# erick093/MPI_Pytorch

Hardware: AMD Instinct MI355X
Metric: images/sec (whole node) ResNet-18 224x224 training at 1/2/4/8 MI355X (higher is better)
Workload: dtype bf16; 1 GPU; model=resnet18, global_batch=2048, per_gpu_batch=2048, image_size=224, num_classes=64500, optimizer=adam, parallelism=dp1, device=cuda, backend=none, hip_graph=False, deterministic=True

## Files before the change

csrc/bindings.cpp:

```cpp
#include <torch/extension.h>
#include <c10/hip/HIPStream.h>
#include <c10/core/DeviceGuard.h>

#include <vector>

#include "kernels/api.h"
#include "runtime/runtime.h"

using torch::Tensor;

namespace {

inline hipStream_t cur_stream() { return c10::hip::getCurrentHIPStream().stream(); }

#define CHECK_CUDA(x) TORCH_CHECK((x).is_cuda(), #x " must be a GPU tensor")
#define CHECK_CONTIG(x) TORCH_CHECK((x).is_contiguous(), #x " must be contiguous")
#define CHECK_BF16(x) \
  TORCH_CHECK((x).scalar_type() == torch::kBFloat16, #x " must be bfloat16, got ", (x).scalar_type())
#define CHECK_F32(x) \
  TORCH_CHECK((x).scalar_type() == torch::kFloat32, #x " must be float32, got ", (x).scalar_type())
#define CHECK_ACT(x) \
  CHECK_CUDA(x);     \
  CHECK_CONTIG(x);   \
  CHECK_BF16(x)
// ... 198 lines not shown
      if (Hp <= 0 || Wp <= 0) continue;
      const int t0 = T;
      for (int r = 0; r < R; ++r) {
        if (((a_ + ph - r) % sh) != 0) continue;
        for (int s = 0; s < S; ++s) {
          if (((b_ + pw - s) % sw) != 0) continue;
          a.taps.dh[T] = (a_ + ph - r) / sh;
          a.taps.dw[T] = (b_ + pw - s) / sw;
          a.taps.bt[T] = r * S + s;
          ++T;
        }
      }
      if (src2) {
        const int R2 = src2->w2.size(1), S2 = src2->w2.size(2);
        for (int r = 0; r < R2; ++r) {
          if (((a_ + src2->ph2 - r) % sh) != 0) continue;
          for (int s = 0; s < S2; ++s) {
            if (((b_ + src2->pw2 - s) % sw) != 0) continue;
            TORCH_CHECK(T < mpa::MAXT, "conv_dgrad: too many taps");
            a.taps.dh[T] = (a_ + src2->ph2 - r) / sh;
            a.taps.dw[T] = (b_ + src2->pw2 - s) / sw;
            a.taps.bt[T] = (short)((r * S2 + s) | mpa::TAP_SRC2);
            ++T;
          }
        }
      }
      TORCH_CHECK(nph < mpa::MAXPH, "conv_dgrad: too many stride phases");
      a.ph[nph++] = mpa::PhaseDesc{N * Hp * Wp, Hp, Wp, (T - t0) * K, t0, T - t0, a_, b_, 0};
    }
  if (bnred) {
    a.ep_z = bp(bnred->z);
    a.ep_y = bopt(bnred->y);
    a.ep_mean = fopt(bnred->mean);
    a.ep_rstd = fopt(bnred->rstd);
    a.ep_gamma = fopt(bnred->gamma);
    a.ep_beta = fopt(bnred->beta);
    TORCH_CHECK(a.ep_y || (a.ep_gamma && a.ep_beta),
                "conv_dgrad_bnred: needs y or gamma / beta for the ReLU mask");
    TORCH_CHECK(!a.ep_gamma == !a.ep_beta, "conv_dgrad_bnred: gamma and beta go together");
    for (const Tensor* t : {&bnred->mean, &bnred->rstd, &bnred->gamma, &bnred->beta})
      TORCH_CHECK(!has(*t) || t->numel() == C, "conv_dgrad_bnred: per-channel vector size");
    bnred->sums = torch::empty({2 * C}, dy.options().dtype(torch::kFloat32));
    int k = 0;
    bool empty = false;
    for (int i = 0; i < nph; ++i) {
      empty |= a.ph[i].T == 0;
      if (a.ph[i].T > 0) a.ph[k++] = a.ph[i];
    }
    if (empty) dx.zero_();
    if (sh == 1 && sw == 1) {
      const mpa::PhaseDesc& d = a.ph[0];
      a.M = d.M; a.oH = d.oH; a.oW = d.oW; a.T = d.T; a.Ktot = d.Ktot; a.Poh = 0; a.Pow = 0;
      a.nphase = 0;
    } else {
      a.nphase = k;
    }
    TORCH_CHECK(!empty, "conv_dgrad_bnred: stride-phase without taps");
    Tensor slab = torch::empty({mpa::igemm_bnred_slab_floats(N * H * W, C, std::max(a.nphase, 1))},
                               dy.options().dtype(torch::kFloat32));
    mpa::igemm_rows_dgrad_bnred(a, vw, bkc, slab.data_ptr<float>(),
                                bnred->sums.data_ptr<float>(), cur_stream());
    return dx;
  }
  if (sh == 1 && sw == 1) {
    const mpa::PhaseDesc& d = a.ph[0];
    a.M = d.M; a.oH = d.oH; a.oW = d.oW; a.T = d.T; a.Ktot = d.Ktot; a.Poh = 0; a.Pow = 0;
    Tensor ws;
    float* wsp = alloc_ws(ws, dy, mpa::igemm_ws_floats(a.M, a.N, a.Ktot));
    mpa::igemm_rows_dgrad(a, vw, wsp, cur_stream(), bkc);
  } else {
    bool empty = false;
    for (int i = 0; i < nph; ++i) empty |= a.ph[i].T == 0;
    int k = 0;
    for (int i = 0; i < nph; ++i)
      if (a.ph[i].T > 0) a.ph[k++] = a.ph[i];
    a.nphase = k;
    if (src2) {
      a.A2 = bp(src2->dy2);
      a.B2 = bp(src2->wt2);
      a.ldb2 = src2->w2.size(1) * src2->w2.size(2) * K;
      if (!mpa::igemm_dgrad_src2_ok(a, vw, bkc)) return Tensor();
    }
    if (empty && !acc) dx.zero_();
    mpa::igemm_rows_dgrad_phases(a, vw, cur_stream(), bkc);
  }
  return dx;
}

Tensor conv_dgrad(Tensor dy, Tensor w, int64_t H, int64_t W, int64_t sh, int64_t sw, int64_t ph,
                  int64_t pw, c10::optional<Tensor> wt_opt, c10::optional<Tensor> accum) {
  return conv_dgrad_impl(dy, w, H, W, sh, sw, ph, pw, wt_opt, nullptr, accum);
}

c10::optional<Tensor> conv_dgrad_res(Tensor dy, Tensor w, Tensor wt, int64_t H, int64_t W,
                                     int64_t ph, int64_t pw, Tensor res, Tensor rmask) {
  CHECK_ACT(dy);
  CHECK_ACT(w);
  CHECK_ACT(res);
  const int N = dy.size(0), P = dy.size(1), Q = dy.size(2), K = dy.size(3);
  const int R = w.size(1), S = w.size(2), C = w.size(3);
  TORCH_CHECK(w.size(0) == K, "conv_dgrad_res: channel mismatch");
  TORCH_CHECK(res.dim() == 4 && res.size(0) == N && res.size(1) == H && res.size(2) == W &&
                  res.size(3) == C,
              "conv_dgrad_res: the residual gradient must have dx's shape");
  TORCH_CHECK(rmask.scalar_type() == torch::kUInt8 && rmask.is_contiguous() &&
                  rmask.numel() == res.numel() / 8 && rmask.device() == res.device(),
              "conv_dgrad_res: ReLU mask must be contiguous uint8 [numel / 8]");
  if (!(wt.defined() && wt.numel() == w.numel()) || vec_width(K) != 8 || vec_width(C) != 8 ||
      mpa::igemm_engine() < 1)
    return c10::nullopt;
  if (P != H + 2 * ph - R + 1 || Q != W + 2 * pw - S + 1) return c10::nullopt;
  if (C % 64 != 0) return c10::nullopt;
  const c10::OptionalDeviceGuard g(device_of(dy));
  Tensor dx = empty_like_shape(dy, {N, H, W, C}, torch::kBFloat16);
  mpa::IGemmArgs a{};
  a.A = bp(dy); a.aH = P; a.aW = Q; a.aC = K;
  a.Uh = 1; a.Uw = 1; a.Oh = 0; a.Ow = 0;
  a.B = bp(wt); a.N = C; a.RS = R * S; a.ldb = R * S * K; a.b_tapmap = 1;
  a.C = dx.data_ptr(); a.ldc = C;
  a.dH = H; a.dW = W; a.Uoh = 1; a.Uow = 1;
  a.beta = 1;
  a.ep_res = bp(res);
  a.ep_rmask = rmask.data_ptr<uint8_t>();
  int T = 0;
  for (int r = 0; r < R; ++r)
    for (int s = 0; s < S; ++s) {
      a.taps.dh[T] = ph - r;
      a.taps.dw[T] = pw - s;
      a.taps.bt[T] = r * S + s;
      ++T;
    }
  a.T = T;
  a.M = N * H * W; a.oH = H; a.oW = W; a.Ktot = T * K; a.Poh = 0; a.Pow = 0;
  if (!mpa::conv3_halo_ok(a)) return c10::nullopt;
  mpa::igemm_rows_dgrad(a, 8, nullptr, cur_stream(), true);
  return dx;
}

c10::optional<Tensor> conv_dgrad_pair(Tensor dy, Tensor w, Tensor wt, int64_t H, int64_t W,
                                      int64_t sh, int64_t sw, int64_t ph, int64_t pw,
                                      Tensor dy2, Tensor w2, Tensor wt2, int64_t ph2,
                                      int64_t pw2, c10::optional<Tensor> accum) {
  CHECK_ACT(dy2);
  CHECK_ACT(w2);
  CHECK_ACT(wt2);
  TORCH_CHECK(dy2.sizes() == dy.sizes(), "conv_dgrad_pair: dy2 must have dy's shape");
  TORCH_CHECK(w2.dim() == 4 && w2.size(0) == w.size(0) && w2.size(3) == w.size(3) &&
                  wt2.numel() == w2.numel(),
              "conv_dgrad_pair: w2 [K][R2][S2][C] with w's K and C, and its transpose");
  if (sh == 1 && sw == 1) return c10::nullopt;
  if (!(wt.defined() && wt.numel() == w.numel())) return c10::nullopt;
  const int P2 = (H + 2 * ph2 - w2.size(1)) / sh + 1, Q2 = (W + 2 * pw2 - w2.size(2)) / sw + 1;
  if (P2 != dy.size(1) || Q2 != dy.size(2)) return c10::nullopt;
  DgradSrc2 s2{dy2, w2, wt2, (int)ph2, (int)pw2};
  Tensor dx = conv_dgrad_impl(dy, w, H, W, sh, sw, ph, pw, wt, nullptr, accum, &s2);
  if (!dx.defined()) return c10::nullopt;
  return dx;
}

bool conv_bnred_ok(int64_t K, int64_t C) {
  return mpa::igemm_engine() >= 1 && vec_width(K) == 8 && vec_width(C) == 8 && C % 8 == 0;
}

std::vector<Tensor> conv_dgrad_bnred(Tensor dy, Tensor w, int64_t H, int64_t W, int64_t sh,
                                     int64_t sw, int64_t ph, int64_t pw, Tensor wt, Tensor z,
                                     Tensor y, Tensor mean, Tensor rstd,
                                     c10::optional<Tensor> gamma, c10::optional<Tensor> beta) {
// ... 1413 lines not shown
  const int64_t ld = src.size(-1);
  TORCH_CHECK(off >= 0 && cs > 0 && off + cs <= ld && (ld * u) % 8 == 0 && (cs * u) % 8 == 0 &&
                  (off * u) % 8 == 0, "chan_slice: 16-byte aligned channel runs required");
  const int64_t rows = src.numel() / ld;
  TORCH_CHECK(rows * (cs * u / 8) < (int64_t(1) << 31), "chan_slice: too large");
  const c10::OptionalDeviceGuard gd(device_of(src));
  std::vector<int64_t> shape(src.sizes().begin(), src.sizes().end());
  shape.back() = cs;
  Tensor out = torch::empty(shape, src.options());
  if (rows > 0)
    mpa::chan_slice((const mpa::bf16_raw*)src.data_ptr(), (int)(ld * u), (int)(off * u),
                    (mpa::bf16_raw*)out.data_ptr(), (int)(cs * u), (int)rows, cur_stream());
  return out;
}

Tensor chan_extract(Tensor g, int64_t off, int64_t cs) {
  CHECK_CUDA(g);
  CHECK_CONTIG(g);
  CHECK_F32(g);
  const int64_t ctot = g.size(-1);
  TORCH_CHECK(ctot % 8 == 0 && cs % 8 == 0 && off % 8 == 0 && off >= 0 && off + cs <= ctot && cs > 0,
              "chan_extract: channel range outside G (multiples of 8 required)");
  const int64_t pixels = g.numel() / ctot;
  TORCH_CHECK(pixels * (cs / 8) < (int64_t(1) << 31), "chan_extract: too large");
  const c10::OptionalDeviceGuard gd(device_of(g));
  std::vector<int64_t> shape(g.sizes().begin(), g.sizes().end());
  shape.back() = cs;
  Tensor out = torch::empty(shape, g.options().dtype(torch::kBFloat16));
  if (pixels > 0)
    mpa::chan_extract(g.data_ptr<float>(), (int)ctot, (int)off, bpm(out), (int)cs, (int)pixels,
                      cur_stream());
  return out;
}

std::vector<Tensor> split_channels(Tensor dy, std::vector<int64_t> sizes) {
  CHECK_ACT(dy);
  TORCH_CHECK(dy.dim() >= 2 && !sizes.empty(), "split_channels: dy must be [..., C]");
  int64_t ctot = 0;
  for (int64_t c : sizes) {
    TORCH_CHECK(c > 0 && c % 8 == 0, "split_channels: channels must be a multiple of 8");
    ctot += c;
  }
  TORCH_CHECK(ctot == dy.size(-1), "split_channels: sizes do not sum to C");
  const int64_t pixels = dy.numel() / ctot;
  TORCH_CHECK(pixels * (ctot / 8) < (int64_t(1) << 31), "split_channels: too large");
  const c10::OptionalDeviceGuard g(device_of(dy));
  std::vector<Tensor> out;
  std::vector<mpa::bf16_raw*> ptrs;
  std::vector<int> chans;
  std::vector<int64_t> shape(dy.sizes().begin(), dy.sizes().end());
  for (int64_t c : sizes) {
    shape.back() = c;
    out.push_back(torch::empty(shape, dy.options()));
    ptrs.push_back(bpm(out.back()));
    chans.push_back((int)c);
  }
  if (pixels > 0)
    mpa::split_channels(bp(dy), chans.data(), (int)sizes.size(), (int)pixels, (int)ctot,
                        ptrs.data(), cur_stream());
  return out;
}

}

extern "C" const char* mpa_src_hash();

PYBIND11_MODULE(TORCH_EXTENSION_NAME, m) {
  m.doc() = "mpi_pytorch_amd native gfx950 kernels + runtime";
  m.def("src_hash", [] { return std::string(mpa_src_hash()); },
        "hash of the csrc/ sources this binary was built from (setup.py source_hash)");
  m.def("igemm_engine", &mpa::igemm_engine, "GEMM staging engine: 1 LDS-DMA, 0 register");
  m.def("igemm_set_engine", &mpa::igemm_set_engine);
  m.def("igemm_force_tile", &mpa::igemm_force_tile, "override GEMM tile (BM, BN, splits); 0 = auto");
  m.def("igemm_set_tune", &mpa::igemm_set_tune, "tile autotuner on/off (MPA_TUNE)");
  m.def("igemm_set_tune_drain", &mpa::igemm_set_tune_drain,
        "tuner candidates: drain the whole device (1, single GPU) or only their stream (0)");
  m.def("set_deterministic", &mpa::set_deterministic,
        "fixed-order reductions + no timing-based autotuning (MPA_DETERMINISTIC)");
  m.def("deterministic", &mpa::deterministic);
  m.def("igemm_tuned_table", &mpa::igemm_tuned_table, "autotuned GEMM tiles so far");
  m.def("igemm_tuned_load", &mpa::igemm_tuned_load, py::arg("table"), py::arg("replace") = true,
        "adopt an igemm_tuned_table() dump (data-parallel ranks take rank 0's)");
  m.def("igemm_set_dma_uni", &mpa::igemm_set_dma_uni, "LDS-DMA uniform-tap fast path on/off");
  m.def("igemm_set_halo", &mpa::igemm_set_halo, "halo-staged direct 3x3/s1 conv on/off");
  m.def("igemm_set_halo_mi7", &mpa::igemm_set_halo_mi7, "448-pixel halo tiles on/off");
  m.def("igemm_set_halo_strip", &mpa::igemm_set_halo_strip,
        "strip-tiled halo conv: 0 off, 1 images too wide for linear tiles, 2 also layer1");
  m.def("igemm_halo_enabled", &mpa::igemm_halo_enabled);
  m.def("igemm_set_stem", &mpa::igemm_set_stem, "direct row-staged 7x7 pixel-pair stem on/off");
  m.def("preprocess_set_copy", &mpa::preprocess_set_copy,
        "identity-size preprocess fast path on/off (MPA_PRE_COPY)");
  m.def("set_comm_reserve", &mpa::set_comm_reserve,
        "CUs held by an overlapping collective (persistent conv grids use the rest)");
  m.def("comm_reserve", &mpa::comm_reserve, "current collective CU reservation");
  m.def("active_cus", &mpa::active_cus, "CUs the persistent conv grids size for");
  m.def("igemm_set_halo_wprod", &mpa::igemm_set_halo_wprod,
        "halo weight gradients on producer-wave blocks on/off (MPA_HALO_WPROD)");
  m.def("igemm_set_halo_wxmap", &mpa::igemm_set_halo_wxmap,
        "XCD-grouped halo weight-gradient block order on/off (MPA_HALO_WXMAP)");
  m.def("igemm_set_halo_trim", &mpa::igemm_set_halo_trim,
        "geometry-sized halo fetch of the linear-tile 3x3 kernels on/off (A/B, tests)");
  m.def("conv3_halo_dma_count", &mpa::conv3_halo_dma_count, py::arg("H"), py::arg("W"),
        "planned halo DMAs per producer wave and item, 256-pixel forward / dgrad tiles");
  m.def("conv3_halo_wgrad_dma_count", &mpa::conv3_halo_wgrad_dma_count, py::arg("H"),
        py::arg("W"), "planned halo DMAs per wave and chunk, 4-wave weight-gradient tiles");
  m.def("affine_act", &affine_act, "relu?(x * aff[0] + aff[1]) per channel (aff [2, C])");
  m.def("conv_fwd", &conv_fwd, py::arg("x"), py::arg("w"), py::arg("bias"), py::arg("sh"),
        py::arg("sw"), py::arg("ph"), py::arg("pw"), py::arg("relu"), py::arg("stats"),
        py::arg("shift"), "conv forward (+ BN statistics of its output)");
  m.def("conv_dgrad", &conv_dgrad, py::arg("dy"), py::arg("w"), py::arg("H"), py::arg("W"),
        py::arg("sh"), py::arg("sw"), py::arg("ph"), py::arg("pw"), py::arg("wt") = py::none(),
        py::arg("accum") = py::none());
  m.def("conv_wgrad", &conv_wgrad, py::arg("dy"), py::arg("x"), py::arg("dw"), py::arg("sh"),
        py::arg("sw"), py::arg("ph"), py::arg("pw"), py::arg("overwrite") = false,
        "weight gradient into dw (+=; overwrite: dw = ..., the first gradient since zero)");
  m.def("conv_bnred_ok", &conv_bnred_ok);
  m.def("conv_dgrad_bnred_gacc", &conv_dgrad_bnred_gacc);
  m.def("conv_dgrad_res", &conv_dgrad_res);
  m.def("conv_dgrad_pair", &conv_dgrad_pair, py::arg("dy"), py::arg("w"), py::arg("wt"),
        py::arg("H"), py::arg("W"), py::arg("sh"), py::arg("sw"), py::arg("ph"), py::arg("pw"),
        py::arg("dy2"), py::arg("w2"), py::arg("wt2"), py::arg("ph2"), py::arg("pw2"),
        py::arg("accum") = py::none());
  m.def("bn_defer_step", &bn_defer_step, py::arg("sums"), py::arg("gamma"), py::arg("mean"),
        py::arg("rstd"), py::arg("s0"), py::arg("k12"), py::arg("dgamma"), py::arg("dbeta"),
        py::arg("G"), py::arg("x"), py::arg("out") = py::none());
  m.def("conv_fwd_into", &conv_fwd_into);
  m.def("conv_dgrad_bnred", &conv_dgrad_bnred, py::arg("dy"), py::arg("w"), py::arg("H"),
        py::arg("W"), py::arg("sh"), py::arg("sw"), py::arg("ph"), py::arg("pw"), py::arg("wt"),
        py::arg("z"), py::arg("y"), py::arg("mean"), py::arg("rstd"),
        py::arg("gamma") = py::none(), py::arg("beta") = py::none());
  m.def("bn_bwd_apply", &bn_bwd_apply);
  m.def("act_bwd", &act_bwd);
  m.def("bn_fwd_train", &bn_fwd_train, py::arg("x"), py::arg("stats"), py::arg("gamma"),
        py::arg("beta"), py::arg("rmean"), py::arg("rvar"), py::arg("momentum"), py::arg("eps"),
        py::arg("res"), py::arg("relu"), py::arg("counter") = py::none(),
        py::arg("mask") = py::none(), py::arg("channels") = 0,
        py::arg("res_affine") = py::none(), py::arg("out") = py::none());
  m.def("bn_stats_affine", &bn_stats_affine, py::arg("x"), py::arg("stats"), py::arg("gamma"),
        py::arg("beta"), py::arg("rmean"), py::arg("rvar"), py::arg("momentum"),
        py::arg("eps"), py::arg("counter") = py::none());
  m.def("bn_stats", &bn_stats, "[mean | biased var] of x [..., C]");
  m.def("bn_relu_avgpool2_fwd", &bn_relu_avgpool2_fwd);
  m.def("bn_fwd_eval", &bn_fwd_eval, py::arg("x"), py::arg("gamma"), py::arg("beta"),
        py::arg("rmean"), py::arg("rvar"), py::arg("eps"), py::arg("res"), py::arg("relu"),
        py::arg("channels") = 0);
  m.def("bn_bwd_pair", &bn_bwd_pair);
  m.def("maxpool_bwd_relu", &maxpool_bwd_relu);
  m.def("bn_bwd", &bn_bwd, py::arg("dy"), py::arg("x"), py::arg("y"), py::arg("mean"),
        py::arg("rstd"), py::arg("gamma"), py::arg("dgamma"), py::arg("dbeta"),
        py::arg("want_dx"), py::arg("want_g"), py::arg("zmask_beta") = py::none(),
        py::arg("ymask") = py::none(), py::arg("gacc") = py::none(),
        py::arg("dx_out") = py::none());
  m.def("relu_fwd", &relu_fwd);
  m.def("comm_emulator", &comm_emulator, "diagnostics: occupy CUs like a concurrent collective");
  m.def("atomic_latency", &atomic_latency, "diagnostics: dependent atomic round trips");
  m.def("maxpool_fwd", &maxpool_fwd);
  m.def("maxpool_bwd", &maxpool_bwd);
  m.def("bn_relu_maxpool_fwd", &bn_relu_maxpool_fwd, py::arg("z"), py::arg("stats"),
        py::arg("gamma"), py::arg("beta"), py::arg("rmean"), py::arg("rvar"), py::arg("momentum"),
        py::arg("eps"), py::arg("kh"), py::arg("kw"), py::arg("sh"), py::arg("sw"), py::arg("ph"),
        py::arg("pw"), py::arg("ceil"), py::arg("counter") = py::none(),
        py::arg("zsel_out") = py::none());
  m.def("maxpool_bn_bwd_sums", &maxpool_bn_bwd_sums);
  m.def("stem_pool_wgrad_ok", &stem_pool_wgrad_ok);
  m.def("stem_pool_wgrad", &stem_pool_wgrad);
  m.def("maxpool_bn_bwd", &maxpool_bn_bwd, py::arg("dp"), py::arg("idx"), py::arg("z"),
// ... 68 lines not shown
```

csrc/kernels/api.h:

```cpp
#pragma once
#include <algorithm>
#include <string>
#include <hip/hip_runtime.h>
#include <stdint.h>

namespace mpa {

typedef uint16_t bf16_raw;
constexpr int MAXT = 128;

struct Taps {
  short dh[MAXT];
  short dw[MAXT];
  short bt[MAXT];
};

struct FastDiv {
  uint32_t m, s;
};
inline FastDiv make_fastdiv(uint32_t d) {
  if (d <= 1) return FastDiv{0u, 0u};
  const uint32_t l = 32u - (uint32_t)__builtin_clz(d - 1u);
  return FastDiv{(uint32_t)(((1ull << (31 + l)) + d - 1) / d), l - 1u};
}

constexpr int MAXPH = 16;
struct PhaseDesc {
  int M, oH, oW, Ktot, tap0, T, Poh, Pow, tiles;
  FastDiv fd_hw, fd_ow;
};

struct IGemmArgs {
  const bf16_raw* A;
  int aH, aW, aC;
  int oH, oW;
  int M;
  int Uh, Uw, Oh, Ow;
  int T;
  int Ktot;
  const bf16_raw* B;
  int N;
  int RS;
  int ldb;
  void* C;
  int ldc;
  int dH, dW, Uoh, Uow, Poh, Pow;
  const float* bias;
  float* stats;
  const float* stats_shift;
  float* stats_sums;
  int stats_ld;
  int relu;
  int ktiles_per_split;
  int tiles_n;
  int tiles_total;
  Taps taps;
  int nphase;
  PhaseDesc ph[MAXPH];
  int b_tapmap;
  int ep_bnred;
  const bf16_raw* ep_z;
  const bf16_raw* ep_y;
  const float* ep_mean;
  const float* ep_rstd;
  const float* ep_gamma;
  const float* ep_beta;
  void* ep_gacc;
  int ep_gacc_f32;
  int stap;
  int beta;
  FastDiv fd_hw, fd_ow;
  const bf16_raw* A2;
  const bf16_raw* B2;
  int ldb2;
  int kpad;
  const bf16_raw* ep_res;
  const uint8_t* ep_rmask;
};
constexpr short TAP_SRC2 = 0x2000;

inline void igemm_set_fastdiv(IGemmArgs& a) {
  a.fd_hw = make_fastdiv((uint32_t)std::max(1, a.oH * a.oW));
  a.fd_ow = make_fastdiv((uint32_t)std::max(1, a.oW));
  for (int i = 0; i < a.nphase && i < MAXPH; ++i) {
    a.ph[i].fd_hw = make_fastdiv((uint32_t)std::max(1, a.ph[i].oH * a.ph[i].oW));
    a.ph[i].fd_ow = make_fastdiv((uint32_t)std::max(1, a.ph[i].oW));
  }
}

struct WGradArgs {
  const bf16_raw* dy;
  const bf16_raw* x;
  float* dw;
  float* slab;
  int Kout, C, H, W, P, Q, R, S, sh, sw, ph, pw;
  int Mpix;
  int Ncols;
  int ktiles_per_split;
  int tiles_n, tiles_total;
  int overwrite;
};

int64_t igemm_slab_floats(int M, int N);
void igemm_rows(IGemmArgs a, int vw, float* ws, float* slab, hipStream_t s);
void igemm_rows_dgrad(IGemmArgs a, int vw, float* ws, hipStream_t s, bool bkc = false);
void igemm_rows_dgrad_phases(IGemmArgs a, int vw, hipStream_t s, bool bkc = false);
bool igemm_dgrad_src2_ok(const IGemmArgs& a, int vw, bool bkc);
int64_t igemm_bnred_slab_floats(int M, int N, int nphase);
void igemm_rows_dgrad_bnred(IGemmArgs a, int vw, bool bkc, float* slab, float* sums,
                            hipStream_t s);
void igemm_wgrad(WGradArgs a, int vwa, int vwb, hipStream_t s);
int64_t igemm_ws_floats(int M, int N, int Ktot);
int64_t igemm_wgrad_ws_floats(int Kout, int Ncols, int Mpix);
int igemm_engine();
void igemm_set_engine(int engine);
void igemm_force_tile(int bm, int bn, int splits);
void igemm_set_tune(int on);
void igemm_set_tune_drain(int on);
std::string igemm_tuned_table();
int igemm_tuned_load(const std::string& table, bool replace);
void igemm_set_dma_uni(int on);
bool igemm_stap_ok();
bool conv3_halo_ok(const IGemmArgs& a);
int conv3_halo(IGemmArgs a, hipStream_t s);
constexpr int HALO_MAX_ROWS = 256;
void igemm_set_halo(int on);
void igemm_set_halo_mi7(int on);
void igemm_set_halo_strip(int mode);
bool stem_wgrad_ok(const WGradArgs& a);
int stem_wgrad(WGradArgs a, hipStream_t s);
int64_t stem_wgrad_ws_floats();
struct StemPoolArgs {
  const bf16_raw* dp;
  const uint8_t* idx;
  const float *mean, *rstd, *gamma, *beta;
  const float* sums;
  int PP, PQ;
  float invM;
};
bool stem_pool_wgrad_ok(const WGradArgs& a, const StemPoolArgs& q);
int stem_pool_wgrad(WGradArgs a, StemPoolArgs q, hipStream_t s);
void igemm_stem_pool_wgrad(WGradArgs a, StemPoolArgs q, hipStream_t s);
bool conv3_halo_wgrad_ok(const WGradArgs& a);
void igemm_set_halo_wxmap(int on);
void igemm_set_halo_wprod(int on);
void igemm_set_halo_trim(int on);
int conv3_halo_dma_count(int H, int W);
int conv3_halo_wgrad_dma_count(int H, int W);
int conv3_halo_wgrad(WGradArgs a, hipStream_t s);
int64_t conv3_halo_wgrad_ws_floats(int Kout, int Ncols);
bool igemm_halo_enabled();
void set_comm_reserve(int cus);
int comm_reserve();
int active_cus();
bool conv_stem_ok(const IGemmArgs& a);
int conv_stem(IGemmArgs a, hipStream_t s);
void igemm_set_stem(int on);

int64_t bn_ws_floats(int M, int C);
void slab_reduce(const float* slab, int S, int W, float* out, bool zero_out, hipStream_t s);
bool dense_gacc_ok(const IGemmArgs& a);
void dense_gacc(IGemmArgs a, float* slab, float* sums, hipStream_t s);
void bn_defer_step(const float* sums, const float* gamma, const float* mean, const float* rstd,
                   int Ci, int s0, int M, float* k12, int ldk, float* dgamma, float* dbeta,
                   void* G, bool g_f32, int ldg, const bf16_raw* x, int ldx, bf16_raw* out,
                   hipStream_t s);
void set_deterministic(int on);
bool deterministic();
void slab_stats(float* slab, int S, int C, const float* shift, int M, float* sums, float* out,
                hipStream_t s, int out_ld = 0);
void stats_finalize(const float* sums, const float* shift, int M, int C, float* out,
                    hipStream_t s);
void bn_stats(const bf16_raw* x, int M, int C, const float* shift, float* stats, float* ws,
              hipStream_t s);
void bn_fwd_train(const bf16_raw* x, const float* stats, const float* gamma, const float* beta,
                  float* rmean, float* rvar, float momentum, float eps, const bf16_raw* res,
                  int relu, int M, int C, bf16_raw* y, float* mean, float* rstd,
                  int64_t* counter, hipStream_t s,
                  uint8_t* ymask = nullptr,
                  int ldx = 0,
                  int lds = 0,
                  const float* res_aff = nullptr,
                  int ldy = 0);
void bn_stats_affine(const float* stats, const float* gamma, const float* beta, float* rmean,
                     float* rvar, float momentum, float eps, int M, int C, float* mean,
                     float* rstd, float* aff, int64_t* counter, hipStream_t s);
void bn_relu_avgpool2_fwd(const bf16_raw* z, const float* aff, int N, int H, int W, int C,
                          bf16_raw* y, hipStream_t s);
void affine_act(const bf16_raw* x, const float* aff, int relu, int M, int C, bf16_raw* y,
                hipStream_t s);
// ... 188 lines not shown
```

csrc/kernels/igemm.hip:

```cpp
#include <algorithm>
#include <cstdio>
#include <cstdlib>
#include <map>
#include <mutex>
#include <string>
#include "igemm_common.h"

namespace mpa {

template <int BM, int BN, int WM, int WN, int VW, bool BKC, bool SPLIT, int OCC>
__global__ __launch_bounds__(256, OCC) void igemm_rows_kernel(IGemmArgs p) {
  constexpr int NA = BM / 64;
  constexpr int A_BYTES = BM * 64;
  constexpr int B_BYTES = BN * 64;
  constexpr int STAGE = A_BYTES + B_BYTES;
  constexpr int TM = BM / WM / 16;
  constexpr int TN = BN / WN / 16;
  constexpr int NB_KC = (BN * 4 + 255) / 256;
  constexpr int CPR = BN / 8;
  constexpr int NB_MN = (BK * CPR + 255) / 256;
  constexpr int NB = BKC ? NB_KC : NB_MN;
  __shared__ __attribute__((aligned(16))) char smem[2 * STAGE];

  const int tid = threadIdx.x;
// ... 855 lines not shown
  a.ep_bnred = 1;
  a.stats = slab;
  a.stats_sums = sums;
  int BM, BN, rows;
  if (a.nphase == 0 && bkc) {
    IGemmArgs t = a;
    if (t.ep_gamma && t.ep_beta) t.ep_y = nullptr;
    if (conv3_halo_ok(t)) {
      rows = conv3_halo(t, s);
      slab_reduce(slab, rows, 2 * a.N, sums, false, s);
      return;
    }
  }
  if (a.nphase > 0) {
    rows = plan_phases(a, BM, BN);
  } else {
    int splits;
    rows_plan(a, BM, BN, splits, false, true);
    rows = (a.M + BM - 1) / BM;
  }
  igemm_rows_dma(a, BM, BN, bkc, 1, s);
  slab_reduce(slab, rows, 2 * a.N, sums, false, s);
}

bool igemm_dgrad_src2_ok(const IGemmArgs& a, int vw, bool bkc) {
  return use_dma(vw) && a.nphase > 0 && a.nphase <= MAXPH && igemm_rows_uni_src2_ok(a, bkc);
}

void igemm_rows_dgrad_phases(IGemmArgs a, int vw, hipStream_t s, bool bkc) {
  a.stats = nullptr;
  a.bias = nullptr;
  if (a.nphase <= 0) return;
  if (a.A2 && !igemm_dgrad_src2_ok(a, vw, bkc)) {
    fprintf(stderr, "igemm_rows_dgrad_phases: second source on an ineligible launch\n");
    abort();
  }
  if (use_dma(vw) && a.nphase <= MAXPH) {
    int tbm = 0, tbn = 0;
    if (g_tune && !deterministic() && !(g_force_bm && g_force_bn) && !stream_capturing(s)) {
      const std::string key = rows_key(a, bkc, false);
      std::unique_lock<std::mutex> pass(g_tune_pass_mu, std::defer_lock);
      if (!tuned_lookup(key, tbm, tbn) && (pass.lock(), !tuned_lookup(key, tbm, tbn))) {
        const int64_t hw0 = std::max(1, a.ph[0].oH * a.ph[0].oW);
        const int64_t rows = (a.ph[0].M + hw0 - 1) / hw0 * a.dH * a.dW;
        const int64_t cbytes = rows * std::max(a.ldc, a.N) * 2;
        char* scr = tune_scratch(cbytes + 256);
        float best = 1e30f;
        for (const auto& c : kRowsCands) {
          if (!scr || !rows_cand_ok(c[0], c[1], a.N)) continue;
          IGemmArgs b = a;
          int BM, BN;
          plan_phases(b, BM, BN, c[0], c[1]);
          if (BM != c[0] || BN != c[1] || b.tiles_total <= 0) continue;
          b.C = scr;
          const float t = time_launches([&] { igemm_rows_dma(b, BM, BN, bkc, 1, s); }, s);
          if (t < best) { best = t; tbm = c[0]; tbn = c[1]; }
        }
        if (tbm) tuned_store(key, tbm, tbn);
      }
    }
    int BM, BN;
    plan_phases(a, BM, BN, tbm, tbn);
    if (a.tiles_total > 0 && igemm_rows_dma(a, BM, BN, bkc, 1, s)) return;
  }
  if (a.A2) {
    fprintf(stderr, "igemm_rows_dgrad_phases: no merged launch for a second source\n");
    abort();
  }
  for (int i = 0; i < a.nphase; ++i) {
    const PhaseDesc& d = a.ph[i];
    IGemmArgs b = a;
    b.nphase = 0;
    b.M = d.M; b.oH = d.oH; b.oW = d.oW; b.Ktot = d.Ktot; b.T = d.T;
    b.Poh = d.Poh; b.Pow = d.Pow;
    for (int t = 0; t < d.T; ++t) {
      b.taps.dh[t] = a.taps.dh[d.tap0 + t];
      b.taps.dw[t] = a.taps.dw[d.tap0 + t];
      b.taps.bt[t] = a.taps.bt[d.tap0 + t];
    }
    run_rows(b, bkc, vw, nullptr, nullptr, s);
  }
}

template <int BM, int BN, int WM, int WN, int VWA, int VWB>
static void launch_wgrad(const WGradArgs& a, int splits, hipStream_t s) {
  dim3 grid(a.tiles_total, 1, splits);
  const int o = occ_target();
  if (o == 4)
    hipLaunchKernelGGL((igemm_wgrad_kernel<BM, BN, WM, WN, VWA, VWB, 4>), grid, dim3(256), 0, s, a);
  else if (o == 2)
    hipLaunchKernelGGL((igemm_wgrad_kernel<BM, BN, WM, WN, VWA, VWB, 2>), grid, dim3(256), 0, s, a);
  else
    hipLaunchKernelGGL((igemm_wgrad_kernel<BM, BN, WM, WN, VWA, VWB, 3>), grid, dim3(256), 0, s, a);
}

template <int BM, int BN>
static void wgrad_vw(const WGradArgs& a, int vwa, int vwb, int splits, hipStream_t s) {
  if (vwb == 1) {
    if (vwa == 8) launch_wgrad<BM, BN, 2, 2, 8, 1>(a, splits, s);
    else if (vwa == 4) launch_wgrad<BM, BN, 2, 2, 4, 1>(a, splits, s);
    else launch_wgrad<BM, BN, 2, 2, 1, 1>(a, splits, s);
  } else {
    if (vwa == 8) launch_wgrad<BM, BN, 2, 2, 8, 8>(a, splits, s);
    else if (vwa == 4) launch_wgrad<BM, BN, 2, 2, 4, 8>(a, splits, s);
    else launch_wgrad<BM, BN, 2, 2, 1, 8>(a, splits, s);
  }
}

static bool wgrad_big(const WGradArgs& a, bool dma_ok) {
  return dma_ok && (a.Kout >= 256 || ((int64_t)a.Kout * a.Ncols <= 32768 && a.Mpix >= (1 << 20)));
}

static bool wgrad_tile_ok(int bm, int bn, bool dma) {
  const bool ok_reg = (bm == 64 || bm == 128) && bn == 128;
  const bool ok_dma = ok_reg || (bn == 256 && (bm == 64 || bm == 128 || bm == 256));
  return dma ? ok_dma : ok_reg;
}

static void wgrad_plan(WGradArgs& a, int& BM, int& BN, int& splits, bool dma, bool big,
                       int tbm = 0, int tbn = 0) {
  BM = (a.Kout <= 64) ? 64 : 128;
  BN = 128;
  if (dma && BM == 128 && ((a.Kout + 127) / 128) * ((a.Ncols + 127) / 128) < 4) BM = 64;
  if (big) BN = 256, BM = (a.Kout <= 64) ? 64 : 128;
  const bool tuned = tbm && tbn && wgrad_tile_ok(tbm, tbn, dma);
  if (tuned) { BM = tbm; BN = tbn; }
  if (g_force_bm && g_force_bn && wgrad_tile_ok(g_force_bm, g_force_bn, dma)) {
    BM = g_force_bm;
    BN = g_force_bn;
  }
  a.tiles_n = (a.Ncols + BN - 1) / BN;
  const int tiles_m = (a.Kout + BM - 1) / BM;
  a.tiles_total = tiles_m * a.tiles_n;
  const int ktiles = (a.Mpix + BK - 1) / BK;
  const bool stem2 = big && BM == 64 && BN == 256 && !(g_force_bm && g_force_bn) && !tuned &&
                     a.Ncols > 128 && a.Ncols <= 256;
  if (stem2) {
    BN = 128;
    a.tiles_n = (a.Ncols + BN - 1) / BN;
    a.tiles_total = tiles_m * a.tiles_n;
  }
  splits = std::max(1, ((stem2 ? 1024 : 512) + a.tiles_total - 1) / a.tiles_total);
  splits = std::min(splits, std::max(1, ktiles / 16));
  if (g_force_splits > 0) splits = std::min(g_force_splits, std::max(ktiles, 1));
  const int64_t out = (int64_t)a.Kout * a.Ncols;
  splits = (int)std::min<int64_t>(splits, std::max<int64_t>(1, (16ll << 20) / out));
  finish_split_plan(ktiles, splits, a.ktiles_per_split);
}

int64_t igemm_wgrad_ws_floats(int Kout, int Ncols, int Mpix) {
  int64_t best = conv3_halo_wgrad_ws_floats(Kout, Ncols);
  if (Kout == 64 && Ncols == 224) best = std::max(best, stem_wgrad_ws_floats());
  for (int dma = 0; dma < 3; ++dma) {
    WGradArgs a{};
    a.Kout = Kout; a.Ncols = Ncols; a.Mpix = Mpix;
    int BM, BN, splits;
    wgrad_plan(a, BM, BN, splits, dma >= 1, dma == 2);
    if (splits > 1) best = std::max(best, (int64_t)splits * Kout * Ncols);
  }
  return best;
}

static void wgrad_run_plan(WGradArgs a, int vwa, int vwb, hipStream_t s, int tbm, int tbn);

void igemm_stem_pool_wgrad(WGradArgs a, StemPoolArgs q, hipStream_t s) {
  const int z = stem_pool_wgrad(a, q, s);
// ... 94 lines not shown
```

csrc/kernels/igemm_common.h:

```cpp
#pragma once
#include "common.h"
#include "api.h"

namespace mpa {

__device__ __forceinline__ u32x4 u32x4_make(uint32_t a, uint32_t b, uint32_t c, uint32_t d) {
  return u32x4{a, b, c, d};
}

constexpr int BK = 32;

__device__ __forceinline__ int kc_off(int row, int chunk) {
  return row * 64 + ((chunk ^ ((4 - ((row >> 2) & 3)) & 3)) << 4);
}

template <int COLS>
__device__ __forceinline__ int mn_swz(int k) {
  if constexpr (COLS >= 128) return 2 * ((k & 3) | (((k >> 3) & 1) << 2));
  else if constexpr (COLS == 64) return 2 * (((k >> 1) & 1) | (((k >> 3) & 1) << 1));
  else return 2 * ((k >> 3) & 1);
}
template <int COLS>
__device__ __forceinline__ int mn_off(int k, int col) {
  const int chunk = col >> 3;
// ... 289 lines not shown
      }
    }
    if (p.stats) {
#pragma unroll
      for (int j = 0; j < TN; ++j)
#pragma unroll
        for (int r = 0; r < 4; ++r) {
          float a = s[j][r], b = q[j][r];
#pragma unroll
          for (int o = 1; o < 16; o <<= 1) {
            a += __shfl_xor(a, o, 64);
            b += __shfl_xor(b, o, 64);
          }
          s[j][r] = a;
          q[j][r] = b;
        }
      float* red = (float*)smem;
      if ((lane & 15) == 0) {
#pragma unroll
        for (int j = 0; j < TN; ++j) {
          const int col = wcol0 + j * 16 + nl;
#pragma unroll
          for (int r = 0; r < 4; ++r) {
            red[(wm * BN + col + r) * 2] = s[j][r];
            red[(wm * BN + col + r) * 2 + 1] = q[j][r];
          }
        }
      }
      __syncthreads();
      if (stat_row == 0 && block_split() == 0 && tid < BN && n0 + tid < p.N) {
        p.stats_sums[n0 + tid] = 0.f;
        p.stats_sums[p.N + n0 + tid] = 0.f;
      }
      if (tid < BN && n0 + tid < p.N) {
        float a = 0.f, b = 0.f;
#pragma unroll
        for (int w = 0; w < WM; ++w) {
          a += red[(w * BN + tid) * 2];
          b += red[(w * BN + tid) * 2 + 1];
        }
        p.stats[(size_t)stat_row * 2 * p.N + n0 + tid] = a;
        p.stats[(size_t)stat_row * 2 * p.N + p.N + n0 + tid] = b;
      }
    }
  }
}

template <int BM, int BN, int WM, int WN>
__device__ __forceinline__ void wgrad_epilogue(const WGradArgs& p,
                                               f32x4 (&acc)[BM / WM / 16][BN / WN / 16],
                                               int m0, int n0, int wrow0, int wcol0,
                                               int lane) {
  constexpr int TM = BM / WM / 16;
  constexpr int TN = BN / WN / 16;
  const int nl = (lane >> 4) * 4;
  const bool direct = gridDim.z == 1;
  const bool vec = (p.Ncols & 3) == 0;
  float* dst = direct ? p.dw : p.slab + (size_t)blockIdx.z * p.Kout * p.Ncols;
#pragma unroll
  for (int i = 0; i < TM; ++i) {
    const int m = m0 + wrow0 + i * 16 + (lane & 15);
    if (m >= p.Kout) continue;
#pragma unroll
    for (int j = 0; j < TN; ++j) {
      const int n = n0 + wcol0 + j * 16 + nl;
      float* q = dst + (size_t)m * p.Ncols + n;
      if (vec && n + 3 < p.Ncols) {
        f32x4 v = acc[i][j];
        if (direct && !p.overwrite) v += *(const f32x4*)q;
        *(f32x4*)q = v;
      } else {
#pragma unroll
        for (int r = 0; r < 4; ++r)
          if (n + r < p.Ncols) q[r] = (direct && !p.overwrite) ? q[r] + acc[i][j][r] : acc[i][j][r];
      }
    }
  }
}

bool igemm_rows_dma(const IGemmArgs& a, int BM, int BN, bool bkc, int splits, hipStream_t s);
bool igemm_rows_uni_src2_ok(const IGemmArgs& a, bool bkc);
bool igemm_rows_kpad_ok(const IGemmArgs& a, bool bkc);
bool igemm_wgrad_dma(const WGradArgs& a, int BM, int BN, int splits, hipStream_t s);
bool igemm_wgrad_inc_ok(const WGradArgs& a);

}
```

csrc/kernels/igemm_dma.hip:

```cpp
#include <algorithm>
#include <cstdlib>
#include <type_traits>
#include "igemm_common.h"

namespace mpa {

static __device__ __attribute__((aligned(16))) uint32_t g_zero16[4];

__device__ __forceinline__ void glds16(const void* src, char* lds_wave_base) {
  __builtin_amdgcn_global_load_lds((const __attribute__((address_space(1))) void*)src,
                                   (__attribute__((address_space(3))) void*)lds_wave_base, 16,
                                   0, 0);
}

template <int N>
__device__ __forceinline__ void wait_barrier() {
  asm volatile("s_waitcnt vmcnt(%0) lgkmcnt(0)\n\ts_barrier" ::"n"(N) : "memory");
}

__device__ __forceinline__ int kc_lane_chunk(int lane) {
  const int sub = lane >> 2;
  return (lane & 3) ^ ((4 - ((sub >> 2) & 3)) & 3);
}

// ... 271 lines not shown
  }

  int t_s = (kbeg * BK) / kpt;
  int c_s = kbeg * BK - t_s * kpt;
  auto issue = [&](uint32_t st) {
    const int hwv = __builtin_amdgcn_readfirstlane(tap_hw[t_s]);
    const int dh = hwv >> 16, dw = (short)(hwv & 0xffff);
    const int toff = __builtin_amdgcn_readfirstlane(tap_ab[t_s]) + c_s * 2;
    const int braw = __builtin_amdgcn_readfirstlane(tap_ab[MAXT + t_s]);
    const bool x2 = PH && BKC && braw < 0;
    const __amdgpu_buffer_rsrc_t rA = x2 ? ra2 : ra;
    const __amdgpu_buffer_rsrc_t rB = x2 ? rb2 : rb;
    const bool cok = !p.kpad || c_s + kch * 8 < aC;
#pragma unroll
    for (int i = 0; i < IAW; ++i) {
      const bool ok = ((unsigned)(a_bh[i] + dh) < (unsigned)p.aH) &
                      ((unsigned)(a_bw[i] + dw) < (unsigned)p.aW) & cok;
      buf_lds16_at(rA, st + (wave * IAW + i) * 1024, ok ? a_off[i] + toff : 0x80000000u);
    }
    const uint32_t bst = st + A_BYTES;
    const int boff = (braw & 0x7fffffff) + (BKC ? c_s * 2 : c_s * p.RS * p.ldb * 2);
    const bool bok = (!p.stap || kch < (__builtin_amdgcn_readfirstlane(tap_b[t_s]) >> 12)) & cok;
#pragma unroll
    for (int i = 0; i < IBW; ++i) {
      const int jb = wave + NW * i;
      uint32_t bo = b_off[i];
      if constexpr (PH && BKC) {
        if (x2) bo = (uint32_t)((min(n0 + 16 * min(jb, IB - 1) + (lane >> 2), p.N - 1) * p.ldb2 +
                                 kch * 8) * 2);
      }
      if (jb < IB) buf_lds16_so(rB, bst + jb * 1024, bok ? bo : 0x80000000u, boff);
    }
    c_s += BK;
    if (c_s >= kpt) { c_s = 0; ++t_s; }
  };

  f32x4 acc[TM][TN];
#pragma unroll
  for (int i = 0; i < TM; ++i)
#pragma unroll
    for (int j = 0; j < TN; ++j) acc[i][j] = f32x4{0.f, 0.f, 0.f, 0.f};
  const int wrow0 = wm * (BM / WM);
  const int wcol0 = wn * (BN / WN);

  auto compute = [&](const char* st) {
    const char* bimg = st + A_BYTES;
    bf16x8 af[TM], bfr[TN];
#pragma unroll
    for (int i = 0; i < TM; ++i) af[i] = frag_kc(st, wrow0 + i * 16 + (lane & 15), lane);
#pragma unroll
    for (int j = 0; j < TN; ++j) {
      if constexpr (BKC) bfr[j] = frag_kc(bimg, wcol0 + j * 16 + (lane & 15), lane);
      else bfr[j] = frag_mn<BN>(bimg, wcol0 + j * 16, lane);
    }
#pragma unroll
    for (int i = 0; i < TM; ++i)
#pragma unroll
      for (int j = 0; j < TN; ++j) acc[i][j] = mfma16(bfr[j], af[i], acc[i][j]);
  };

  if (kbeg < kend) {
    issue(s32);
    if (kbeg + 1 < kend) issue(s32 + STAGE);
    int kt = kbeg;
    auto step = [&](auto sc) {
      constexpr int S = decltype(sc)::value;
      if (kt + 1 < kend) wait_barrier<WAITN>();
      else wait_barrier<0>();
      if (kt + 2 < kend) issue(s32 + ((S + 2) % 3) * STAGE);
      compute(smem + S * STAGE);
      ++kt;
    };
    while (kt + 3 <= kend) {
      step(std::integral_constant<int, 0>{});
      step(std::integral_constant<int, 1>{});
      step(std::integral_constant<int, 2>{});
    }
    if (kt < kend) step(std::integral_constant<int, 0>{});
    if (kt < kend) step(std::integral_constant<int, 1>{});
  }
  __syncthreads();
  rows_epilogue<BM, BN, WM, WN, SPLIT>(p, acc, smem, mt, m0, n0, wm, wrow0, wcol0, tid, g,
                                       row_base + mt);
}

template <int BM, int BN, int WM, int WN>
__global__ __launch_bounds__(WM * WN * 64, dma_occ(3 * (BM + BN) * 64, WM * WN))
void igemm_wgrad_dma_kernel(WGradArgs p) {
  constexpr int NW = WM * WN;
  constexpr int NS = 3;
  constexpr int A_BYTES = BK * BM * 2, B_BYTES = BK * BN * 2, STAGE = A_BYTES + B_BYTES;
  constexpr int CPRA = BM / 8, RPIA = 64 / CPRA;
  constexpr int CPRB = BN / 8, RPIB = 64 / CPRB;
  constexpr int IA = BM / 16, IB = BN / 16;
  constexpr int IAW = (IA + NW - 1) / NW, IBW = (IB + NW - 1) / NW;
  constexpr int WAITN = IA / NW + IB / NW;
  constexpr int TM = BM / WM / 16;
  constexpr int TN = BN / WN / 16;
  static_assert(NW == 4 || NW == 8, "tile");
  __shared__ __attribute__((aligned(16))) char smem[NS * STAGE];

  const int tid = threadIdx.x;
  const int lane = tid & 63;
  const int wave = tid >> 6;
  const int wm = wave / WN, wn = wave % WN;

  const int tile = xcd_remap(blockIdx.x, p.tiles_total);
  const int mt = tile / p.tiles_n, nt = tile % p.tiles_n;
  const int m0 = mt * BM, n0 = nt * BN;
  const int ktiles = (p.Mpix + BK - 1) / BK;
  const int kbeg = blockIdx.z * p.ktiles_per_split;
  const int kend = min(ktiles, kbeg + p.ktiles_per_split);
  if (kbeg >= kend) return;
  const bf16_t* const zp = (const bf16_t*)g_zero16;

  int a_row[IAW], a_m[IAW];
#pragma unroll
  for (int i = 0; i < IAW; ++i) {
    const int ja = wave + NW * i;
    a_row[i] = RPIA * ja + lane / CPRA;
    a_m[i] = m0 + (((lane % CPRA) ^ mn_swz<BM>(a_row[i])) << 3);
  }
  const int PQ = p.P * p.Q;
  int b_dh[IBW], b_dw[IBW], b_c[IBW], b_img[IBW], b_oh[IBW], b_ow[IBW];
  bool b_ok[IBW];
#pragma unroll
  for (int i = 0; i < IBW; ++i) {
    const int jb = wave + NW * i;
    const int krow = RPIB * jb + lane / CPRB;
    const int n = n0 + (((lane % CPRB) ^ mn_swz<BN>(krow)) << 3);
    const int tap = n / p.C;
    const int r = tap / p.S;
    b_dh[i] = r - p.ph;
    b_dw[i] = tap - r * p.S - p.pw;
    b_c[i] = n - tap * p.C;
    b_ok[i] = n < p.Ncols;
    const int pix = kbeg * BK + krow;
    const int img = pix / PQ;
    const int rr = pix - img * PQ;
    b_img[i] = img;
    b_oh[i] = rr / p.Q;
    b_ow[i] = rr - b_oh[i] * p.Q;
  }

  auto issue = [&](int kt, int stage) {
    char* st = smem + stage * STAGE;
#pragma unroll
    for (int i = 0; i < IAW; ++i) {
      const int ja = wave + NW * i;
      if (ja < IA) {
        const int pix = kt * BK + a_row[i];
        const bool ok = (pix < p.Mpix) & (a_m[i] < p.Kout);
        const bf16_t* src = ok ? p.dy + (size_t)pix * p.Kout + a_m[i] : zp;
        glds16(src, st + ja * 1024);
      }
    }
    char* bimg = st + A_BYTES;
#pragma unroll
    for (int i = 0; i < IBW; ++i) {
      const int jb = wave + NW * i;
      if (jb < IB) {
        const int pix = kt * BK + RPIB * jb + lane / CPRB;
        const int ih = b_oh[i] * p.sh + b_dh[i], iw = b_ow[i] * p.sw + b_dw[i];
        const bool ok = b_ok[i] & (pix < p.Mpix) & ((unsigned)ih < (unsigned)p.H) &
                        ((unsigned)iw < (unsigned)p.W);
        const bf16_t* src =
// ... 298 lines not shown
```

Measured before the change: 57900 images/sec.

## Add cell-form 3x3 stride-2 dgrad kernel computing all four output phases per tile

Adds a dedicated kernel for the stride-2, pad-1, 3x3 conv data gradient. Each output tile covers 2x2 cells of input pixels and computes all four stride phases at once. Every dy tap-shifted A tile is loaded once and reused across the phases that need it, instead of being restaged per phase by the merged-phase rows kernel. It is enabled by default and falls back when the tap plan does not match, at the cost of a new kernel with larger accumulator state and an LDS-staged scatter epilogue.

Result: no change. 58360 images/sec, median of 6 (+0.8%).

```diff
diff --git a/csrc/bindings.cpp b/csrc/bindings.cpp
--- a/csrc/bindings.cpp
+++ b/csrc/bindings.cpp
@@ -304,7 +304,8 @@
       if (!mpa::igemm_dgrad_src2_ok(a, vw, bkc)) return Tensor();
     }
     if (empty && !acc) dx.zero_();
-    mpa::igemm_rows_dgrad_phases(a, vw, cur_stream(), bkc);
+    if (!empty && mpa::igemm_dgrad_cells_ok(a, vw, bkc)) mpa::igemm_dgrad_cells(a, cur_stream());
+    else mpa::igemm_rows_dgrad_phases(a, vw, cur_stream(), bkc);
   }
   return dx;
 }
@@ -1884,6 +1885,10 @@
   m.def("igemm_tuned_load", &mpa::igemm_tuned_load, py::arg("table"), py::arg("replace") = true,
         "adopt an igemm_tuned_table() dump (data-parallel ranks take rank 0's)");
   m.def("igemm_set_dma_uni", &mpa::igemm_set_dma_uni, "LDS-DMA uniform-tap fast path on/off");
+  m.def("set_dgrad_cells", &mpa::igemm_set_dgrad_cells,
+        "cell form of the 3x3/s2/p1 dgrad on/off (off: merged stride phases)");
+  m.def("dgrad_cells_count", &mpa::igemm_dgrad_cells_count,
+        "launches of the cell-form dgrad so far");
   m.def("igemm_set_halo", &mpa::igemm_set_halo, "halo-staged direct 3x3/s1 conv on/off");
   m.def("igemm_set_halo_mi7", &mpa::igemm_set_halo_mi7, "448-pixel halo tiles on/off");
   m.def("igemm_set_halo_strip", &mpa::igemm_set_halo_strip,
diff --git a/csrc/kernels/api.h b/csrc/kernels/api.h
--- a/csrc/kernels/api.h
+++ b/csrc/kernels/api.h
@@ -106,6 +106,10 @@
 void igemm_rows_dgrad(IGemmArgs a, int vw, float* ws, hipStream_t s, bool bkc = false);
 void igemm_rows_dgrad_phases(IGemmArgs a, int vw, hipStream_t s, bool bkc = false);
 bool igemm_dgrad_src2_ok(const IGemmArgs& a, int vw, bool bkc);
+bool igemm_dgrad_cells_ok(const IGemmArgs& a, int vw, bool bkc);
+void igemm_dgrad_cells(const IGemmArgs& a, hipStream_t s);
+void igemm_set_dgrad_cells(int on);
+int64_t igemm_dgrad_cells_count();
 int64_t igemm_bnred_slab_floats(int M, int N, int nphase);
 void igemm_rows_dgrad_bnred(IGemmArgs a, int vw, bool bkc, float* slab, float* sums,
                             hipStream_t s);
diff --git a/csrc/kernels/igemm.hip b/csrc/kernels/igemm.hip
--- a/csrc/kernels/igemm.hip
+++ b/csrc/kernels/igemm.hip
@@ -961,6 +961,70 @@
   }
 }
 
+static bool g_dgrad_cells = [] {
+  const char* e = getenv("MPA_DGRAD_CELLS");
+  return !(e && e[0] == '0');
+}();
+static int64_t g_dgrad_cells_count = 0;
+void igemm_set_dgrad_cells(int on) { g_dgrad_cells = on != 0; }
+int64_t igemm_dgrad_cells_count() { return g_dgrad_cells_count; }
+
+static bool cells_plan_matches(const IGemmArgs& a) {
+  if (a.nphase != 4 || a.Uh != 1 || a.Uw != 1 || a.Oh != 0 || a.Ow != 0 || a.Uoh != 2 ||
+      a.Uow != 2 || a.RS != 9 || a.dH != 2 * a.aH || a.dW != 2 * a.aW || a.ldc != a.N)
+    return false;
+  for (int f = 0; f < 4; ++f) {
+    const PhaseDesc& d = a.ph[f];
+    if (d.Poh != (f >> 1) || d.Pow != (f & 1) || d.oH != a.aH || d.oW != a.aW ||
+        d.M != a.ph[0].M || d.M % (a.aH * a.aW) != 0)
+      return false;
+    int t = d.tap0;
+    for (int e = 0; e < CELL_SEGS; ++e)
+      for (int q = 0; q < cell_nact(e); ++q) {
+        if (cell_phase(e, q) != f) continue;
+        if (t >= d.tap0 + d.T || a.taps.dh[t] != cell_dh(e) || a.taps.dw[t] != cell_dw(e) ||
+            a.taps.bt[t] != cell_tap(e, q))
+          return false;
+        ++t;
+      }
+    if (f == 0 && a.A2) {
+      if (t >= d.tap0 + d.T || a.taps.dh[t] != 0 || a.taps.dw[t] != 0 ||
+          a.taps.bt[t] != TAP_SRC2)
+        return false;
+      ++t;
+    }
+    if (t != d.tap0 + d.T || d.Ktot != d.T * a.aC) return false;
+  }
+  return true;
+}
+
+bool igemm_dgrad_cells_ok(const IGemmArgs& a, int vw, bool bkc) {
+  if (!g_dgrad_cells || !use_dma(vw) || !igemm_stap_ok() || !bkc || !a.b_tapmap || a.beta || a.ep_bnred ||
+      a.ep_res || a.stap || a.kpad || a.relu)
+    return false;
+  if (a.aC % BK != 0 || a.N % 64 != 0 || !cells_plan_matches(a)) return false;
+  if (a.A2 ? !(a.B2 && a.ldb2 == a.aC) : a.B2 != nullptr) return false;
+  if (a.ldb != 9 * a.aC) return false;
+  const int64_t cells = a.ph[0].M;
+  return cells * a.aC * 2 < (1ll << 31) && (int64_t)a.N * a.ldb * 2 < (1ll << 31) &&
+         cells * 4 < (1ll << 31);
+}
+
+void igemm_dgrad_cells(const IGemmArgs& a, hipStream_t s) {
+  DgradCellArgs c{};
+  c.A = a.A; c.A2 = a.A2; c.B = a.B; c.B2 = a.B2;
+  c.C = (bf16_raw*)a.C;
+  c.P = a.aH; c.Q = a.aW; c.K = a.aC; c.Cn = a.N;
+  c.M = a.ph[0].M;
+  c.tiles_n = a.N / 64;
+  c.tiles_total = (c.M + CELL_BM - 1) / CELL_BM * c.tiles_n;
+  c.fd_pq = make_fastdiv((uint32_t)(c.P * c.Q));
+  c.fd_q = make_fastdiv((uint32_t)c.Q);
+  if (c.tiles_total <= 0) return;
+  ++g_dgrad_cells_count;
+  igemm_dgrad_cells_launch(c, s);
+}
+
 template <int BM, int BN, int WM, int WN, int VWA, int VWB>
 static void launch_wgrad(const WGradArgs& a, int splits, hipStream_t s) {
   dim3 grid(a.tiles_total, 1, splits);
diff --git a/csrc/kernels/igemm_common.h b/csrc/kernels/igemm_common.h
--- a/csrc/kernels/igemm_common.h
+++ b/csrc/kernels/igemm_common.h
@@ -395,6 +395,32 @@
 bool igemm_rows_uni_src2_ok(const IGemmArgs& a, bool bkc);
 bool igemm_rows_kpad_ok(const IGemmArgs& a, bool bkc);
 bool igemm_wgrad_dma(const WGradArgs& a, int BM, int BN, int splits, hipStream_t s);
+
+constexpr int CELL_SEGS = 5;
+constexpr int cell_dh(int e) { return e < 2 ? 1 : 0; }
+constexpr int cell_dw(int e) { return (e == 0 || e == 2) ? 1 : 0; }
+constexpr int cell_nact(int e) { return (e == 0 || e == 5) ? 1 : 2; }
+constexpr int cell_phase(int e, int q) {
+  return e == 0 ? 3 : e == 1 ? 2 + q : e == 2 ? 1 + 2 * q : e == 3 ? q : e == 4 ? 2 + q : 0;
+}
+constexpr int cell_tap(int e, int q) {
+  return e == 5 ? 0
+                : ((cell_phase(e, q) >> 1) + 1 - 2 * cell_dh(e)) * 3 +
+                      ((cell_phase(e, q) & 1) + 1 - 2 * cell_dw(e));
+}
+struct DgradCellArgs {
+  const bf16_raw* A;
+  const bf16_raw* A2;
+  const bf16_raw* B;
+  const bf16_raw* B2;
+  bf16_raw* C;
+  int P, Q, K, Cn;
+  int M;
+  int tiles_n, tiles_total;
+  FastDiv fd_pq, fd_q;
+};
+constexpr int CELL_BM = 128;
+void igemm_dgrad_cells_launch(const DgradCellArgs& a, hipStream_t s);
 bool igemm_wgrad_inc_ok(const WGradArgs& a);
 
 }
diff --git a/csrc/kernels/igemm_dma.hip b/csrc/kernels/igemm_dma.hip
--- a/csrc/kernels/igemm_dma.hip
+++ b/csrc/kernels/igemm_dma.hip
@@ -377,6 +377,180 @@
   __syncthreads();
   rows_epilogue<BM, BN, WM, WN, SPLIT>(p, acc, smem, mt, m0, n0, wm, wrow0, wcol0, tid, g,
                                        row_base + mt);
+}
+
+template <int BM, int WM, int WN>
+__global__ __launch_bounds__(WM * WN * 64, dma_occ(3 * (BM + 128) * 64, WM * WN))
+void dgrad_cells_kernel(DgradCellArgs p) {
+  constexpr int NW = WM * WN, NT = NW * 64;
+  constexpr int CS = 64;
+  constexpr int A_BYTES = BM * 64, B_BYTES = 2 * CS * 64, STAGE = A_BYTES + B_BYTES;
+  constexpr int IAW = BM / 16 / NW;
+  constexpr int TM = BM / WM / 16;
+  constexpr int FP = CS / WN / 16;
+  constexpr int TN = 4 * FP;
+  constexpr int OROW = 4 * CS * 2 + 16;
+  static_assert(NW * 16 == CS && BM % (16 * NW) == 0 && FP >= 1, "tile");
+  static_assert(BM / WM * OROW + BM * 4 <= 3 * STAGE, "epilogue image fits the ring");
+  __shared__ __attribute__((aligned(16))) char smem[3 * STAGE];
+
+  const int tid = threadIdx.x;
+  const int lane = tid & 63;
+  const int wave = __builtin_amdgcn_readfirstlane(tid >> 6);
+  const int wm = wave / WN, wn = wave % WN;
+  const int tile = xcd_remap(blockIdx.x, p.tiles_total);
+  const int mt = tile / p.tiles_n, nt = tile % p.tiles_n;
+  const int m0 = mt * BM, c0 = nt * CS;
+  const int K = p.K, Q = p.Q;
+  const int ksteps = K / BK;
+  const int total = (p.A2 ? CELL_SEGS + 1 : CELL_SEGS) * ksteps;
+
+  const __amdgpu_buffer_rsrc_t ra = make_rsrc(p.A, 0x7fffffffu);
+  const __amdgpu_buffer_rsrc_t rb = make_rsrc(p.B, 0x7fffffffu);
+  const __amdgpu_buffer_rsrc_t ra2 = make_rsrc(p.A2 ? p.A2 : p.A, 0x7fffffffu);
+  const __amdgpu_buffer_rsrc_t rb2 = make_rsrc(p.B2 ? p.B2 : p.B, 0x7fffffffu);
+  const uint32_t s32 = lds_base(smem);
+  const int kch = kc_lane_chunk(lane);
+
+  uint32_t a_off[IAW];
+  bool a_h1[IAW], a_w1[IAW];
+#pragma unroll
+  for (int i = 0; i < IAW; ++i) {
+    const int m = min(m0 + 16 * (wave * IAW + i) + (lane >> 2), p.M - 1);
+    const int img = (int)fdiv((uint32_t)m, p.fd_pq);
+    const int r = m - img * p.P * Q;
+    const int ci = (int)fdiv((uint32_t)r, p.fd_q);
+    a_h1[i] = ci + 1 < p.P;
+    a_w1[i] = (r - ci * Q) + 1 < Q;
+    a_off[i] = (uint32_t)((m * K + kch * 8) * 2);
+  }
+  const int brow = c0 + 16 * wave + (lane >> 2);
+  const uint32_t b_off = (uint32_t)((brow * 9 * K + kch * 8) * 2);
+  const uint32_t b2_off = (uint32_t)((brow * K + kch * 8) * 2);
+
+  auto issue = [&](auto dc, uint32_t st, int c_s) {
+    constexpr int D = decltype(dc)::value;
+    constexpr int DH = cell_dh(D), DW = cell_dw(D);
+    const int toff = ((DH * Q + DW) * K + c_s) * 2;
+#pragma unroll
+    for (int i = 0; i < IAW; ++i) {
+      const bool ok = (!DH || a_h1[i]) & (!DW || a_w1[i]);
+      buf_lds16_at(D == 5 ? ra2 : ra, st + (wave * IAW + i) * 1024,
+                   ok ? a_off[i] + toff : 0x80000000u);
+    }
+#pragma unroll
+    for (int q = 0; q < cell_nact(D); ++q)
+      buf_lds16_so(D == 5 ? rb2 : rb, st + A_BYTES + (q * NW + wave) * 1024,
+                   D == 5 ? b2_off : b_off, (cell_tap(D, q) * K + c_s) * 2);
+  };
+  int is_d = 0, is_c = 0;
+  auto issue_next = [&](uint32_t st) {
+    switch (is_d) {
+      case 0: issue(std::integral_constant<int, 0>{}, st, is_c); break;
+      case 1: issue(std::integral_constant<int, 1>{}, st, is_c); break;
+      case 2: issue(std::integral_constant<int, 2>{}, st, is_c); break;
+      case 3: issue(std::integral_constant<int, 3>{}, st, is_c); break;
+      case 4: issue(std::integral_constant<int, 4>{}, st, is_c); break;
+      default: issue(std::integral_constant<int, 5>{}, st, is_c); break;
+    }
+    is_c += BK;
+    if (is_c >= K) { is_c = 0; ++is_d; }
+  };
+
+  f32x4 acc[TM][TN];
+#pragma unroll
+  for (int i = 0; i < TM; ++i)
+#pragma unroll
+    for (int j = 0; j < TN; ++j) acc[i][j] = f32x4{0.f, 0.f, 0.f, 0.f};
+  const int wrow0 = wm * (BM / WM);
+  const int wcol0 = wn * (CS / WN);
+  const int a_lds = kc_off(wrow0 + (lane & 15), lane >> 4);
+  const int b_lds = A_BYTES + kc_off(wcol0 + (lane & 15), lane >> 4);
+
+  int t = 0, s = 0;
+  auto run_seg = [&](auto dc) {
+    constexpr int D = decltype(dc)::value;
+    constexpr int NA = cell_nact(D);
+    for (int kc = 0; kc < ksteps; ++kc) {
+      if (t + 1 >= total) wait_barrier<0>();
+      else if (kc + 1 < ksteps) wait_barrier<IAW + NA>();
+      else wait_barrier<IAW + cell_nact(D < 5 ? D + 1 : 5)>();
+      if (t + 2 < total) issue_next(s32 + (s == 0 ? 2 : s - 1) * STAGE);
+      const char* st = smem + s * STAGE;
+      bf16x8 af[TM];
+#pragma unroll
+      for (int i = 0; i < TM; ++i)
+        af[i] = __builtin_bit_cast(bf16x8, *LDS_PTR(const u32x4, st + a_lds + i * 1024));
+#pragma unroll
+      for (int q = 0; q < NA; ++q) {
+#pragma unroll
+        for (int jj = 0; jj < FP; ++jj) {
+          const bf16x8 bfr = __builtin_bit_cast(
+              bf16x8, *LDS_PTR(const u32x4, st + b_lds + (q * CS + jj * 16) * 64));
+          const int j = cell_phase(D, q) * FP + jj;
+#pragma unroll
+          for (int i = 0; i < TM; ++i) acc[i][j] = mfma16(bfr, af[i], acc[i][j]);
+        }
+      }
+      ++t;
+      s = s == 2 ? 0 : s + 1;
+    }
+  };
+
+  issue_next(s32);
+  if (total > 1) issue_next(s32 + STAGE);
+  run_seg(std::integral_constant<int, 0>{});
+  run_seg(std::integral_constant<int, 1>{});
+  run_seg(std::integral_constant<int, 2>{});
+  run_seg(std::integral_constant<int, 3>{});
+  run_seg(std::integral_constant<int, 4>{});
+  if (p.A2) run_seg(std::integral_constant<int, 5>{});
+  __syncthreads();
+
+  constexpr int HR = BM / WM;
+  int* rowpix = (int*)(smem + HR * OROW);
+  for (int r = tid; r < BM; r += NT) {
+    const int m = m0 + r;
+    int pix = -1;
+    if (m < p.M) {
+      const int img = (int)fdiv((uint32_t)m, p.fd_pq);
+      const int rr = m - img * p.P * Q;
+      const int ci = (int)fdiv((uint32_t)rr, p.fd_q);
+      pix = ((img * p.P + ci) * 2 * Q + (rr - ci * Q)) * 2;
+    }
+    rowpix[r] = pix;
+  }
+  const int nl = (lane >> 4) * 4;
+  bf16_t* out = (bf16_t*)p.C;
+  const int W = 2 * Q;
+#pragma unroll
+  for (int h = 0; h < WM; ++h) {
+    if (wm == h) {
+#pragma unroll
+      for (int i = 0; i < TM; ++i) {
+        char* orow = smem + (i * 16 + (lane & 15)) * OROW + (wcol0 + nl) * 2;
+#pragma unroll
+        for (int j = 0; j < TN; ++j) {
+          const f32x4 v = acc[i][j] + 0.f + 0.f;
+          *(uint2*)(orow + (j / FP) * (CS * 2) + (j % FP) * 32) =
+              make_uint2(pack2(v[0], v[1]), pack2(v[2], v[3]));
+        }
+      }
+    }
+    __syncthreads();
+    for (int id = tid; id < HR * 32; id += NT) {
+      const int r = id >> 5, f = (id >> 3) & 3, ch = id & 7;
+      const int pix = rowpix[h * HR + r];
+      if (pix < 0) continue;
+      const uint4 v = *(const uint4*)(smem + r * OROW + f * (CS * 2) + ch * 16);
+      *(uint4*)(out + (size_t)(pix + (f >> 1) * W + (f & 1)) * p.Cn + c0 + ch * 8) = v;
+    }
+    if (h + 1 < WM) __syncthreads();
+  }
+}
+
+void igemm_dgrad_cells_launch(const DgradCellArgs& a, hipStream_t s) {
+  hipLaunchKernelGGL((dgrad_cells_kernel<CELL_BM, 2, 2>), dim3(a.tiles_total), dim3(256), 0, s, a);
 }
 
 template <int BM, int BN, int WM, int WN>
```
